# miniufo/xcontour

Measured on AMD Instinct MI355X. Metric: lat-lon cells*contours/s, full Keff pipeline, higher is better.
Workload: dtype f64

## Files before the change

### xcontour_amd/csrc/xc_capi.h

```cpp
#pragma once
#include "xc_internal.h"
#include <assert.h>

namespace xc {

inline size_t al(size_t x) { return (x + 255) & ~(size_t)255; }
inline size_t esize(int dtype) { return dtype == XC_F32 ? 4 : 8; }
inline size_t dA_bytes(int rank, int64_t nslab, int64_t ny, int64_t nx)
{
    return rank == XC_DA_ROW ? (size_t)ny * 8 : rank == XC_DA_PLANE ? (size_t)ny * nx * 8 : rank == XC_DA_SLAB ? (size_t)nslab * ny * nx * 8 : 0;
}

#define XC_TRY(expr) do { int _rc = (expr); if (_rc != XC_OK) return _rc; } while (0)
#define XC_CTX(ctx) do { if (!(ctx)) return xc::fail(nullptr, XC_EBADARG, "null context"); \
                         hipError_t _e = hipSetDevice((ctx)->device); \
                         if (_e != hipSuccess) return xc::hipfail((ctx), _e, "hipSetDevice"); } while (0)

int grow(xc_ctx* ctx, void** p, size_t* have, size_t need);
void mm_touch(xc_ctx* ctx, const void* p, size_t bytes);
const void* resident_lookup(const xc_ctx* ctx, const void* h, size_t n);
int hist_ev_begin(xc_ctx* ctx);
int hist_ev_end(xc_ctx* ctx);

int h2d(xc_ctx* ctx, void* d, const void* h, size_t n);
int stage_in(xc_ctx* ctx, void* slot, const void* h, size_t n, const void** dev);
int stage_small(xc_ctx* ctx, void* slot, const void* h, size_t n, const void** dev);
int flush_in(xc_ctx* ctx);
int d2h(xc_ctx* ctx, void* h, const void* d, size_t n);
void* out_direct(xc_ctx* ctx, void* h, size_t n);

struct Stage {
    struct Out { void* host; const void* dev; size_t bytes; };
// ... 16 lines not shown
```

### xcontour_amd/csrc/xc_comm.hip

```cpp
#include "xc_internal.h"
#include <dlfcn.h>
#include <string.h>

namespace xc {
namespace {

struct UniqueId { char internal[128]; };
typedef void* Comm;
typedef int (*fn_get_id)(UniqueId*);
typedef int (*fn_init_rank)(Comm*, int, UniqueId, int);
typedef int (*fn_allgather)(const void*, void*, size_t, int , Comm, hipStream_t);
typedef int (*fn_destroy)(Comm);
typedef const char* (*fn_errstr)(int);
typedef int (*fn_sendrecv)(void*, size_t, int , int , Comm, hipStream_t);
typedef int (*fn_group)(void);
typedef int (*fn_comm_int)(const Comm, int*);
typedef int (*fn_version)(int*);

struct Rccl {
    void* h = nullptr;
    fn_get_id get_id = nullptr; fn_init_rank init_rank = nullptr; fn_allgather allgather = nullptr;
    fn_destroy destroy = nullptr; fn_errstr errstr = nullptr;
    fn_sendrecv send = nullptr, recv = nullptr; fn_group group_start = nullptr, group_end = nullptr; fn_destroy abort = nullptr;
    fn_comm_int count = nullptr, user_rank = nullptr, cu_device = nullptr; fn_version version = nullptr;
// ... 47 lines not shown
{
    if (ctx->comm_stream) return XC_OK;
    XC_HIP(ctx, hipStreamCreateWithFlags(&ctx->comm_stream, hipStreamNonBlocking));
    XC_HIP(ctx, hipEventCreateWithFlags(&ctx->ev_comm_in, hipEventDisableTiming));
    XC_HIP(ctx, hipEventCreateWithFlags(&ctx->ev_comm_out, hipEventDisableTiming));
    return XC_OK;
}

}
}

using namespace xc;

#define XC_COMM_CTX(ctx) do { if (!(ctx)) return fail(nullptr, XC_EBADARG, "null context"); \
                              hipError_t _e = hipSetDevice((ctx)->device); \
                              if (_e != hipSuccess) return hipfail((ctx), _e, "hipSetDevice"); } while (0)

extern "C" {

int xc_comm_unique_id(xc_ctx* ctx, void* out_id128)
{
    if (!ctx || !out_id128) return fail(ctx, XC_EBADARG, "xc_comm_unique_id: bad arguments");
    int rc = load_rccl(ctx); if (rc != XC_OK) return rc;
    UniqueId id;
    const int r = g_rccl.get_id(&id);
    if (r != 0) return rccl_fail(ctx, r, "ncclGetUniqueId");
    memcpy(out_id128, &id, sizeof(id));
    return XC_OK;
}

int xc_comm_create(int device, int nranks, int rank, const void* id128, void** out_comm, char* err, size_t errlen)
// ... 61 lines not shown
    }
    if (!ctx->comm) return XC_OK;
    int v = 0;
    if (g_rccl.count && g_rccl.count(ctx->comm, &v) == 0) out->comm_count = v;
    if (g_rccl.user_rank && g_rccl.user_rank(ctx->comm, &v) == 0) out->comm_rank = v;
    if (g_rccl.cu_device && g_rccl.cu_device(ctx->comm, &v) == 0) out->comm_device = v;
    return XC_OK;
}

int xc_comm_allgather_dev(xc_ctx* ctx, const void* send, void* recv, size_t bytes_per_rank)
{
    if (!ctx || !ctx->comm) return fail(ctx, XC_EBADARG, "xc_comm_allgather: no communicator (call xc_comm_init)");
    if (!send || !recv) return fail(ctx, XC_EBADARG, "xc_comm_allgather: NULL buffer");
    hipError_t e = hipSetDevice(ctx->device);
    if (e != hipSuccess) return hipfail(ctx, e, "hipSetDevice");
    const int r = g_rccl.allgather(send, recv, bytes_per_rank, 0 , ctx->comm, ctx->stream);
    if (r != 0) return rccl_fail(ctx, r, "ncclAllGather");
    return XC_OK;
}

int xc_comm_gather_dev(xc_ctx* ctx, const void* send, size_t bytes, void* recv, size_t rank_stride, int root)
{
    XC_COMM_CTX(ctx);
    if (!ctx->comm) return fail(ctx, XC_EBADARG, "xc_comm_gather: no communicator (call xc_comm_init)");
    if (!g_rccl.send || !g_rccl.recv || !g_rccl.group_start || !g_rccl.group_end)
        return fail(ctx, XC_EHIP, "xc_comm_gather: librccl lacks ncclSend / ncclRecv / ncclGroupStart / ncclGroupEnd");
    if (!send || root < 0 || root >= ctx->comm_nranks || (ctx->comm_rank == root && !recv) || rank_stride < bytes)
        return fail(ctx, XC_EBADARG, "xc_comm_gather: bad arguments");
    { const int rc = ensure_comm_stream(ctx); if (rc != XC_OK) return rc; }
    if (bytes == 0) return XC_OK;
// ... 97 lines not shown

int xc_comm_abort(xc_ctx* ctx)
{
    if (!ctx) return fail(nullptr, XC_EBADARG, "null context");
    if (ctx->comm) {
        Comm c = ctx->comm; ctx->comm = nullptr;
        if (g_rccl.abort) { const int r = g_rccl.abort(c); if (r != 0) return rccl_fail(ctx, r, "ncclCommAbort"); }
    }
    return XC_OK;
}

int xc_comm_finalize(xc_ctx* ctx)
{
    if (!ctx) return fail(nullptr, XC_EBADARG, "null context");
    if (ctx->comm) {
        (void)hipStreamSynchronize(ctx->stream);
        if (ctx->comm_stream) (void)hipStreamSynchronize(ctx->comm_stream);
        const int r = g_rccl.destroy(ctx->comm);
        ctx->comm = nullptr;
        if (r != 0) return rccl_fail(ctx, r, "ncclCommDestroy");
    }
    return XC_OK;
}

}
```

### xcontour_amd/csrc/xc_context.hip

```cpp
#include "xc_capi.h"
#include <string.h>
#include <stdio.h>
#include <stdlib.h>
#include <new>
#include <mutex>
#include <set>
#include <utility>

namespace xc {

static thread_local std::string g_err;

int fail(xc_ctx* ctx, int code, const std::string& msg)
{
    if (ctx) {
        ctx->err = msg;
        ctx->pending_out.clear(); ctx->pending_in.clear(); ctx->pin_in_off = 0; ctx->pin_out_off = 0;
        for (auto& e : ctx->small_in) if (e.epoch == ctx->small_epoch) { e.host.clear(); e.epoch = ~0ull; }
        ++ctx->small_epoch;
    } else g_err = msg;
    return code;
}

int hipfail(xc_ctx* ctx, hipError_t e, const char* what)
{
    std::string m = std::string("HIP error: ") + hipGetErrorString(e) + " in " + what;
    (void)hipGetLastError();
    return fail(ctx, e == hipErrorOutOfMemory ? XC_ENOMEM : XC_EHIP, m);
}

int grow(xc_ctx* ctx, void** p, size_t* have, size_t need)
{
    if (need <= *have) return XC_OK;
    size_t want = *have ? *have : (size_t)1 << 20;
    while (want < need) want *= 2;
    if (*p) {
        XC_HIP(ctx, hipStreamSynchronize(ctx->stream));
        XC_HIP(ctx, hipFree(*p));
        *p = nullptr; *have = 0;
    }
    hipError_t e = hipMalloc(p, want);
    if (e != hipSuccess) { want = need; e = hipMalloc(p, want); }
    if (e != hipSuccess) return hipfail(ctx, e, "hipMalloc(scratch)");
    *have = want;
    return XC_OK;
}

int ensure_scratch(xc_ctx* ctx, size_t bytes) { return grow(ctx, &ctx->scratch, &ctx->scratch_bytes, bytes); }
int ensure_arena(xc_ctx* ctx, size_t bytes)   { return grow(ctx, &ctx->arena, &ctx->arena_bytes, bytes); }
int ensure_big(xc_ctx* ctx, size_t bytes)     { return grow(ctx, &ctx->big, &ctx->big_bytes, bytes); }

int ensure_ones(xc_ctx* ctx, size_t n)
// ... 94 lines not shown
    }
    if (strncmp(prop.gcnArchName, "gfx950", 6) != 0) {
        std::string m = std::string("xc_create: device is ") + prop.gcnArchName + ", this library is built for gfx950 only";
        delete ctx; return fail(nullptr, XC_ENODEV, m);
    }
    snprintf(ctx->name, sizeof(ctx->name), "%s (%s, %d CUs, %.0f GB)", prop.name[0] ? prop.name : "AMD Instinct [name not reported by the driver]",
             prop.gcnArchName, prop.multiProcessorCount, (double)prop.totalGlobalMem / 1e9);
    {
        auto env_int = [](const char* name, int dflt) { const char* e = getenv(name); return e ? atoi(e) : dflt; };
        HistKnobs& k = ctx->knobs;
        k.xcd_map = env_int("XC_HIST_XCDMAP", 1); k.tile_map = env_int("XC_HIST_TILEMAP", 1); k.vec4 = env_int("XC_HIST_VEC4", -1); k.e32 = env_int("XC_HIST_E32", 1);
        k.threads = env_int("XC_HIST_THREADS", 0); k.ncopy = env_int("XC_HIST_NCOPY", 0); k.rows = env_int("XC_HIST_ROWS", 0);
        k.bps = env_int("XC_HIST_BPS", 0);
        k.cross_ncopy = env_int("XC_CROSS_NCOPY", 0); k.cross_blocks = env_int("XC_CROSS_BLOCKS", 0);
        k.copy_kernel = env_int("XC_COPY_KERNEL", 1); k.copy_out_kb = env_int("XC_COPY_OUT_KB", 256); if (k.copy_out_kb < 1 || k.copy_out_kb > 1024) k.copy_out_kb = 256; k.single = env_int("XC_KEFF_SINGLE", 1); k.single_timeout_us = env_int("XC_KEFF_SINGLE_TIMEOUT_US", 50000); k.single_map = env_int("XC_KEFF_SINGLE_MAP", 0);
        k.sort_range = env_int("XC_SORT_RANGE", 1); k.lwa_fast = env_int("XC_LWA_FAST", 1); k.k1_nt = env_int("XC_K1_NT", 0); k.lwa_strip = env_int("XC_LWA_STRIP", 1);
    }
    ctx->cus = prop.multiProcessorCount;
    if ((e = hipStreamCreateWithFlags(&ctx->stream, hipStreamNonBlocking)) != hipSuccess) {
        int rc = hipfail(nullptr, e, "hipStreamCreate"); delete ctx; return rc;
    }
    if ((e = hipStreamCreateWithFlags(&ctx->copy_stream, hipStreamNonBlocking)) != hipSuccess ||
        (e = hipEventCreateWithFlags(&ctx->ev_copy, hipEventDisableTiming)) != hipSuccess ||
        (e = hipEventCreateWithFlags(&ctx->ev_compute, hipEventDisableTiming)) != hipSuccess) {
        int rc = hipfail(nullptr, e, "hipStreamCreate(copy)"); delete ctx; return rc;
    }
    if ((e = hipEventCreate(&ctx->ev_hist0)) != hipSuccess || (e = hipEventCreate(&ctx->ev_hist1)) != hipSuccess) {
        int rc = hipfail(nullptr, e, "hipEventCreate"); delete ctx; return rc;
    }
    *out = ctx;
    return XC_OK;
}

int xc_destroy(xc_ctx* ctx)
{
    if (!ctx) return XC_OK;
    (void)hipSetDevice(ctx->device);
    (void)xc_comm_finalize(ctx);
    if (ctx->copy_stream) (void)hipStreamSynchronize(ctx->copy_stream);
    if (ctx->stream) (void)hipStreamSynchronize(ctx->stream);
    if (ctx->comm_stream) { (void)hipStreamSynchronize(ctx->comm_stream); (void)hipStreamDestroy(ctx->comm_stream); }
    if (ctx->ev_comm_in) (void)hipEventDestroy(ctx->ev_comm_in);
    if (ctx->ev_comm_out) (void)hipEventDestroy(ctx->ev_comm_out);
    if (ctx->pinned_flag) (void)hipHostFree(ctx->pinned_flag);
    for (auto& e : ctx->small_in) if (e.dev) (void)hipFree(e.dev);
    if (ctx->pin_in) (void)hipHostFree(ctx->pin_in);
    if (ctx->pin_out) (void)hipHostFree(ctx->pin_out);
    if (ctx->lwa_flag) (void)hipFree(ctx->lwa_flag);
    if (ctx->single_ws) (void)hipFree(ctx->single_ws);
    if (ctx->single_stamps) (void)hipFree(ctx->single_stamps);
    for (auto& e : ctx->resident) (void)hipFree(e.dev);
    if (ctx->ev_copy) (void)hipEventDestroy(ctx->ev_copy);
    if (ctx->ev_compute) (void)hipEventDestroy(ctx->ev_compute);
    if (ctx->copy_stream) (void)hipStreamDestroy(ctx->copy_stream);
    if (ctx->scratch) (void)hipFree(ctx->scratch);
// ... 10 lines not shown

int xc_device_name(xc_ctx* ctx, char* buf, size_t buflen)
{
    if (!ctx || !buf || buflen == 0) return fail(ctx, XC_EBADARG, "xc_device_name: bad arguments");
    snprintf(buf, buflen, "%s", ctx->name);
    return XC_OK;
}

int xc_device_cus(xc_ctx* ctx, int* out_cus)
{
    if (!ctx || !out_cus) return fail(ctx, XC_EBADARG, "xc_device_cus: bad arguments");
    *out_cus = ctx->cus;
    return XC_OK;
}

void* xc_stream(xc_ctx* ctx) { return ctx ? (void*)ctx->stream : nullptr; }

int xc_malloc(xc_ctx* ctx, size_t bytes, void** out_dptr)
{
    XC_CTX(ctx);
    if (!out_dptr) return fail(ctx, XC_EBADARG, "xc_malloc: out is NULL");
    *out_dptr = nullptr;
    XC_HIP(ctx, hipMalloc(out_dptr, bytes ? bytes : 1));
    return XC_OK;
}

int xc_keep_resident(xc_ctx* ctx, const void* host_ptr, size_t bytes)
{
    XC_CTX(ctx);
    if (!host_ptr || bytes == 0) return fail(ctx, XC_EBADARG, "xc_keep_resident: bad arguments");
    XC_HIP(ctx, hipStreamSynchronize(ctx->copy_stream));
// ... 192 lines not shown
```

### xcontour_amd/csrc/xc_forms.hip

```cpp
#include "xc_capi.h"
#include <cmath>

using namespace xc;

static bool check_ascending(const double* contours, int64_t nc, int ncont)
{
    for (int64_t s = 0; s < nc; ++s)
        for (int k = 0; k < ncont; ++k) {
            const double c = contours[s * ncont + k];
            if (c != c || (k > 0 && c < contours[s * ncont + k - 1])) return false;
        }
    return true;
}

static int clen_recorded(xc_ctx* ctx, int rc)
{
    if (rc != XC_OK) ctx->last_clen = xc_clen_geometry{};
    return rc;
}

static int contour_lengths_host(xc_ctx* ctx, const void* q, int q_dtype, int64_t nslab, int64_t ny, int64_t nx,
                                const double* ycoord, const double* xcoord, double radius,
                                const double* contours, int ncont, int contours_per_slab,
                                double* out_len, uint64_t* out_nseg)
// ... 299 lines not shown

int xc_set_lwa_exact(xc_ctx* ctx, int exact)
{
    if (!ctx) return fail(nullptr, XC_EBADARG, "null context");
    if (exact < 0 || exact > 3) return fail(ctx, XC_EBADARG, "xc_set_lwa_exact: mode must be 0 (automatic), 1 (band walk), 2 (interval kernel, checked) or 3 (interval kernel, premises vouched for)");
    ctx->lwa_exact = exact;
    return XC_OK;
}

int xc_last_lwa_path(xc_ctx* ctx, int* out_path)
{
    if (!ctx || !out_path) return fail(ctx, XC_EBADARG, "xc_last_lwa_path: bad arguments");
    if (ctx->last_lwa_path < 0) {
        unsigned f = 0;
        XC_HIP(ctx, hipSetDevice(ctx->device));
        XC_HIP(ctx, hipMemcpyAsync(&f, ctx->lwa_flag, sizeof(f), hipMemcpyDeviceToHost, ctx->stream));
        XC_HIP(ctx, hipStreamSynchronize(ctx->stream));
        ctx->last_lwa_path = (f == ctx->lwa_epoch) ? 2 : 1;
    }
    *out_path = ctx->last_lwa_path;
    return XC_OK;
}

int xc_last_sort_path(xc_ctx* ctx, int* out_path)
{
    if (!ctx || !out_path) return fail(ctx, XC_EBADARG, "xc_last_sort_path: bad arguments");
    *out_path = ctx->last_sort_path;
    return XC_OK;
}

// ... 10 lines not shown
```

### xcontour_amd/csrc/xc_hist_det.hip

```cpp
#include "xc_internal.h"

namespace xc {

namespace {

#include "xc_hist_kernel.h"

template <typename TQ, int VEC, int NINT, bool GRAD>
int det3_two(xc_ctx* ctx, const HistGeom& g, int64_t nslab, const HistArgs& a)
{
    const bool da2d = a.dA_rank == XC_DA_PLANE || a.dA_rank == XC_DA_SLAB;
    if constexpr (GRAD && NINT == 0 && VEC == 2) {
        if (da2d && a.periodic_x && a.dA_pos_finite && !a.negate && !a.last_closed)
            return a.q_next ? launch_three<TQ, VEC, NINT, GRAD, true, true, true, 3>(ctx, g, nslab, a)
                            : launch_three<TQ, VEC, NINT, GRAD, true, false, true, 3>(ctx, g, nslab, a);
    }
    if constexpr ((GRAD && NINT == 0) || (!GRAD && NINT == 1)) {
        if (a.q_next)
            return da2d ? launch_three<TQ, VEC, NINT, GRAD, true, true, false, 3>(ctx, g, nslab, a)
                        : launch_three<TQ, VEC, NINT, GRAD, false, true, false, 3>(ctx, g, nslab, a);
    }
    if (a.q_next) return fail(ctx, XC_EBADARG, "xc_hist: q_next rides in the Keff layouts only");
    return da2d ? launch_three<TQ, VEC, NINT, GRAD, true, false, false, 3>(ctx, g, nslab, a)
                : launch_three<TQ, VEC, NINT, GRAD, false, false, false, 3>(ctx, g, nslab, a);
// ... 55 lines not shown

}

int det_limbs_total(int nch) { return det_total_limbs(nch); }

int launch_hist_det3(xc_ctx* ctx, int q_dtype, int nint, int grad, const HistGeom& g, int64_t nslab, const HistArgs& a)
{
    if (g.vec == 4) return fail(ctx, XC_EBADARG, "xc_hist: no four-cell variant with deterministic sums");
    if (!a.part_c || !a.det_c0_out) return fail(ctx, XC_EBADARG, "xc_hist: the one-pass deterministic sums need the count partials and the window constants");
    if (q_dtype == XC_F64) return g.vec == 2 ? det3_one<double, 2>(ctx, nint, grad, g, nslab, a) : det3_one<double, 1>(ctx, nint, grad, g, nslab, a);
    if (q_dtype == XC_F32) return g.vec == 2 ? det3_one<float, 2>(ctx, nint, grad, g, nslab, a) : det3_one<float, 1>(ctx, nint, grad, g, nslab, a);
    return fail(ctx, XC_EBADARG, "xc_hist: q_dtype must be XC_F32 or XC_F64");
}

int launch_det3_reduce(xc_ctx* ctx, int64_t nslab, int bps, int nch, int nbin, const double* part_l, const unsigned* part_c,
                       const int* c0, double* red_h, unsigned long long* red_c)
{
    dim3 grid((unsigned)((nch * nbin + 7) / 8), (unsigned)nslab);
    hipLaunchKernelGGL(k_det3_reduce, grid, dim3(256), 0, ctx->stream, reinterpret_cast<const unsigned long long*>(part_l), part_c,
                       bps, nch, nbin, c0, red_h, red_c);
    XC_HIP(ctx, hipGetLastError());
    return XC_OK;
}

}
```

### xcontour_amd/csrc/xc_internal.h

```cpp
#pragma once
#include <hip/hip_runtime.h>
#include <stdint.h>
#include <stddef.h>
#include <string>
#include <type_traits>
#include <vector>
#include "../../include/xcontour_hip.h"

struct HistKnobs {
    int copy_out_kb = 256;
    int copy_kernel = 1;
    int xcd_map = 1;
    int tile_map = 1;
    int vec4 = -1;
    int e32 = 1;
    int threads = 0;
    int ncopy = 0;
    int rows = 0;
    int bps = 0;
    int cross_ncopy = 0, cross_blocks = 0;
    int k1_nt = 0;
    int lwa_fast = 1;
    int lwa_strip = 1;
    int sort_range = 1;
    int single = 1;
    int single_timeout_us = 50000;
    int single_map = 0;
};

struct xc_ctx {
    int device = 0;
    HistKnobs knobs;
    hipStream_t stream = nullptr;
    hipStream_t copy_stream = nullptr;
    hipStream_t comm_stream = nullptr;
    hipEvent_t ev_comm_in = nullptr, ev_comm_out = nullptr;
    hipEvent_t ev_copy = nullptr, ev_compute = nullptr;
    unsigned* pinned_flag = nullptr;
    char* pin_in = nullptr;  size_t pin_in_off = 0;
    char* pin_out = nullptr; size_t pin_out_off = 0;
    struct PendingOut { void* host; const void* pinned; size_t bytes; const void* dev; };
    std::vector<PendingOut> pending_out;
// ... 8 lines not shown
    int cus = 0;
    char name[256] = {0};
    std::string err;
    void*  scratch = nullptr;   size_t scratch_bytes = 0;
    void*  arena = nullptr;     size_t arena_bytes = 0;
    double* ones = nullptr;     size_t ones_n = 0;
    void*  big = nullptr;       size_t big_bytes = 0;
    int timing = 0;
    hipEvent_t ev_hist0 = nullptr, ev_hist1 = nullptr;
    int ev_valid = 0;
    void* comm = nullptr; int comm_nranks = 0, comm_rank = 0;
    hipEvent_t user_ev0 = nullptr, user_ev1 = nullptr;
    double* mmnext[2] = {nullptr, nullptr};  size_t mmnext_bytes[2] = {0, 0};
    int mm_cur = 0, mm_valid = 0, mm_P = 0, mm_dtype = 0;
    const void* mm_q = nullptr;  int64_t mm_nslab = 0, mm_ny = 0, mm_nx = 0;  int mm_gen = 0;
    int lwa_exact = 0;
    int last_lwa_path = 0;
    unsigned lwa_epoch = 0;
    unsigned* lwa_flag = nullptr;
    int last_sort_path = 0;
    void* single_ws = nullptr;  unsigned single_launches = 0;  int single_dirty_bins[2] = {0, 0};
    int last_keff_path = 0;
    xc_hist_variant last_hist = {};
    xc_clen_geometry last_clen = {};
    unsigned long long* single_stamps = nullptr;
};

namespace xc {

int fail(xc_ctx* ctx, int code, const std::string& msg);
int ensure_big_lds(xc_ctx* ctx, const void* kernel, int bytes);
int hipfail(xc_ctx* ctx, hipError_t e, const char* what);

#define XC_HIP(ctx, call)                                                     \
    do {                                                                      \
        hipError_t _e = (call);                                               \
        if (_e != hipSuccess) return xc::hipfail((ctx), _e, #call);           \
    } while (0)

int ensure_scratch(xc_ctx* ctx, size_t bytes);
int ensure_arena(xc_ctx* ctx, size_t bytes);
int ensure_ones(xc_ctx* ctx, size_t n);
int ensure_big(xc_ctx* ctx, size_t bytes);

constexpr int kMinmaxBlocks = 2048;
// ... 130 lines not shown
                     int dA_rank, SingleGeom* g);
int launch_keff_single(xc_ctx* ctx, int q_dtype, const SingleArgs& a, const SingleGeom& g);

int launch_minmax_partial(xc_ctx* ctx, const void* q, int q_dtype, int64_t nslab, int64_t ncell, double* part,
                          double* zero = nullptr, int64_t nzero = 0, bool finite_only = false);
struct SmallCopies { const void* src[8]; void* dst[8]; unsigned bytes[8]; };
int launch_copy_small(xc_ctx* ctx, const SmallCopies& c, int count);
int launch_minmax_final(xc_ctx* ctx, const double* part, int64_t nslab, int P, double* out);
int launch_levels(xc_ctx* ctx, const double* minmax, int q_dtype, int64_t nslab, int N, int increase,
                  int ctr_dtype, int right_edge, double* ctr, double* edges, int32_t* status, int P = 0, double* minmax_out = nullptr);
int hist_geometry(xc_ctx* ctx, int q_dtype, int64_t nslab, int64_t ny, int64_t nx, int nbin, int nch,
                  const void* q, HistGeom* g, int keff_fast_layout = 0, int det = 0);
int launch_hist(xc_ctx* ctx, int q_dtype, int nint, int grad, const HistGeom& g, int64_t nslab, const HistArgs& a);
int launch_hist_det3(xc_ctx* ctx, int q_dtype, int nint, int grad, const HistGeom& g, int64_t nslab, const HistArgs& a);
int launch_det3_reduce(xc_ctx* ctx, int64_t nslab, int bps, int nch, int nbin, const double* part_l, const unsigned* part_c,
                       const int* c0, double* red_h, unsigned long long* red_c);
int det_limbs_total(int nch);
int launch_finalize(xc_ctx* ctx, int64_t nslab, const FinalArgs& a);
int launch_rowsum(xc_ctx* ctx, const void* mask, int mask_dtype, const double* dA, int dA_rank,
                  int64_t ny, int64_t nx, int multiply, double* out_rows);
int launch_grad2(xc_ctx* ctx, const void* q, int q_dtype, int64_t nslab, int64_t ny, int64_t nx,
                 const double* rdx, const double* rdy, int periodic_x, double* out);
int launch_lwa(xc_ctx* ctx, const void* q, int q_dtype, const double* Q, const double* coord,
               const double* dA, int dA_rank, double dA_max, const double* M, int M_rank,
               int64_t nslab, int64_t ny, int64_t nx, int increase, int part, int variant,
               const int32_t* mask_idx, int nmask, double* out_lwa, int8_t* out_masks);
size_t sort_workspace_bytes(int64_t n, int64_t nslab);
struct SortArgs {
    const void*   q;     int q_dtype;
    const void*   mask;  int mask_dtype, mask_per_slab;
    const double* dA;    int dA_rank;
    int64_t       nslab, ny, nx;
    int           negate;
// ... 23 lines not shown
```

### xcontour_amd/csrc/xc_keff.hip

```cpp
#include "xc_capi.h"
#include <string.h>

using namespace xc;

static const void* vec_align_bits(const void* q, int q_dtype, const void* q_next, const double* dA, int dA_rank,
                                  const void* const* integ, const int32_t* integ_dtype, int nint)
{
    uintptr_t bits = reinterpret_cast<uintptr_t>(q) | reinterpret_cast<uintptr_t>(q_next);
    auto need16 = [&](const void* p) {
        const uintptr_t a = reinterpret_cast<uintptr_t>(p);
        if (a % 16 != 0) bits |= (q_dtype == XC_F32) ? 4 : 8;
    };
    if (dA && (dA_rank == XC_DA_PLANE || dA_rank == XC_DA_SLAB)) need16(dA);
    for (int i = 0; i < nint; ++i) {
        if (integ_dtype[i] == XC_F64) need16(integ[i]);
        else if (reinterpret_cast<uintptr_t>(integ[i]) % 8 != 0) bits |= (q_dtype == XC_F32) ? 4 : 8;
    }
    return reinterpret_cast<const void*>(bits);
}

static int check_hist_desc(xc_ctx* ctx, const xc_hist_desc* d)
{
    if (!d) return fail(ctx, XC_EBADARG, "xc_hist: desc is NULL");
    if (!d->q || !d->edges) return fail(ctx, XC_EBADARG, "xc_hist: q / edges is NULL");
// ... 17 lines not shown
    size_t o_ph, o_pc, o_rh, o_rc, o_c0, o_dp, o_dm, pair_bytes, total = 0;  char* base = nullptr;
    size_t put(size_t bytes) { const size_t at = total; total += al(bytes); return at; }
    K3Scratch(int64_t nslab, int bps, int nch, int nbin, int det, bool minmax_partials, bool part_h = true)
    {
        const size_t S = (size_t)nslab, mmb = S * kMinmaxBlocks * 2 * sizeof(double);
        put(minmax_partials ? mmb : 0);
        o_ph = put(part_h ? S * bps * (det ? det_limbs_total(nch) : nch) * nbin * sizeof(double) : 0);
        o_pc = put(S * bps * nbin * sizeof(unsigned));
        o_rh = put(S * nch * nbin * sizeof(double));
        o_rc = put(S * nbin * sizeof(unsigned long long));
        o_c0 = put(det ? S * nch * sizeof(int) : 0);
        o_dp = put(det ? mmb : 0);
        pair_bytes = al(S * 2 * sizeof(double));
        o_dm = put(det ? (3 + XC_MAX_INTEGRANDS) * pair_bytes : 0);
    }
    int reserve(xc_ctx* ctx) { XC_TRY(ensure_scratch(ctx, total)); base = (char*)ctx->scratch; return XC_OK; }
    double*   mmpart() const { return (double*)base; }
    double*   part_h() const { return (double*)(base + o_ph); }
    unsigned* part_c() const { return (unsigned*)(base + o_pc); }
    size_t    part_c_bytes() const { return o_rh - o_pc; }
    double*   red_h() const  { return (double*)(base + o_rh); }
    unsigned long long* red_c() const { return (unsigned long long*)(base + o_rc); }
    int64_t   acc_words() const { return (int64_t)((o_c0 - o_rh) / 8); }
    int*      c0() const     { return (int*)(base + o_c0); }
    double*   det_part() const { return (double*)(base + o_dp); }
    double*   det_pair(int i) const { return (double*)(base + o_dm + i * pair_bytes); }
};

template <typename Desc, typename Args>
static int set_weights(xc_ctx* ctx, const Desc* d, Args& a)
{
// ... 18 lines not shown
    return XC_OK;
}

static void keff_final(FinalArgs& f, const xc_keff_desc* d, int vstride, int ntbl)
{
    f.lt = d->lt; f.reverse = !d->increase;
    f.keff = 1; f.ctr_f32 = d->ctr_dtype == XC_F32; f.ctr = d->ctr; f.vstride = vstride;
    f.tbl = d->tbl; f.tbl_coord = d->tbl_coord; f.ntbl = ntbl;
    f.preY = d->preY; f.npre = d->interp ? d->npre : 0;
    f.nkeff_mask = d->nkeff_mask; f.lmin_scale = d->lmin_scale;
    f.o_area = d->area; f.o_intS = d->intgrdS; f.o_latEq = d->latEq; f.o_dqdA = d->dqdA; f.o_dSdA = d->dintSdA;
    f.o_Leq2 = d->Leq2; f.o_Lmin = d->Lmin; f.o_nkeff = d->nkeff; f.o_interp = d->interp;
}

static int det_one_pass(xc_ctx* ctx, int q_dtype, int nint, int grad, const HistGeom& g, int64_t nslab, int64_t ny, int64_t nx,
                        HistArgs& a, const K3Scratch& L, double dA_max_host, const void* const* integ, const int* integ_dtype, FinalArgs& f)
{
    double* part = L.det_part();
    auto extrema = [&](const void* p, int dtype, int64_t ns, int64_t ncell, double* out) -> int {
        XC_TRY(launch_minmax_partial(ctx, p, dtype, ns, ncell, part, nullptr, 0, true));
        return launch_minmax_final(ctx, part, ns, minmax_blocks(ncell, ns), out);
    };
    a.det_dA_max = -1.0; a.det_dA_max_dev = nullptr; a.det_dA_stride = 0;
    if (dA_max_host > 0.0 && dA_max_host < __builtin_inf()) a.det_dA_max = dA_max_host;
    else if (a.dA == ctx->ones) a.det_dA_max = 1.0;
    else {
        double* out = L.det_pair(0);
        const int64_t ns = a.dA_rank == XC_DA_SLAB ? nslab : 1, ncell = a.dA_rank == XC_DA_ROW ? ny : ny * nx;
        XC_TRY(extrema(a.dA, XC_F64, ns, ncell, out));
        a.det_dA_max_dev = out; a.det_dA_stride = a.dA_rank == XC_DA_SLAB ? 1 : 0;
    }
    a.det_q_mm = nullptr;
    if (grad && !a.levels_mode) {
        double* out = L.det_pair(1);
        XC_TRY(extrema(a.q, q_dtype, nslab, ny * nx, out));
        a.det_q_mm = out;
    }
    for (int i = 0; i < nint; ++i) {
        double* out = L.det_pair(2 + i);
        XC_TRY(extrema(integ[i], integ_dtype[i], nslab, ny * nx, out));
        a.det_int_mm[i] = out;
    }
    a.det_c0_out = L.c0();
    XC_TRY(launch_hist_det3(ctx, q_dtype, nint, grad, g, nslab, a));
    XC_TRY(launch_det3_reduce(ctx, nslab, g.bps, f.nch, f.nbin, a.part_h, a.part_c, L.c0(), f.red_h, f.red_c));
    f.skip_reduce = 1;
    return XC_OK;
}

static int hist_recorded(xc_ctx* ctx, int rc)
{
    if (rc != XC_OK && ctx) ctx->last_hist = xc_hist_variant{};
    return rc;
}

static int hist_dev(xc_ctx* ctx, const xc_hist_desc* d)
{
    XC_TRY(check_hist_desc(ctx, d));
    const int nbin = (int)(d->nedge - 1), nch = 1 + d->nint + (d->grad ? 1 : 0);
    HistGeom g;
// ... 91 lines not shown
    keff_final(f, d, vstride, (int)d->ny);
    f.abort_flag = &a.cur->abort; f.status_out = d->status;
    f.dbg = ctx->single_stamps ? ctx->single_stamps + 8 : nullptr;
    ctx->mm_valid = 0;
    XC_TRY(hist_ev_begin(ctx));
    XC_TRY(launch_keff_single(ctx, d->q_dtype, a, g));
    XC_TRY(hist_ev_end(ctx));
    XC_TRY(launch_finalize(ctx, d->nslab, f));
    ctx->single_dirty_bins[cur] = N;
    ctx->single_dirty_bins[1u - cur] = 0;
    ++ctx->single_launches;
    ctx->last_keff_path = 1;
    return XC_OK;
}

static int keff_dev(xc_ctx* ctx, const xc_keff_desc* d)
{
    if (!d) return fail(ctx, XC_EBADARG, "xc_keff: desc is NULL");
    if (!d->q || !d->ctr || !d->area || !d->tbl || !d->tbl_coord) return fail(ctx, XC_EBADARG, "xc_keff: q/ctr/area/tbl/tbl_coord must be given");
    if (d->q_dtype != XC_F32 && d->q_dtype != XC_F64) return fail(ctx, XC_EBADARG, "xc_keff: bad q_dtype");
    if (d->ctr_dtype != XC_F32 && d->ctr_dtype != XC_F64) return fail(ctx, XC_EBADARG, "xc_keff: bad ctr_dtype");
    if (d->nslab < 1 || d->ny < 2 || d->nx < 1 || d->N < 2) return fail(ctx, XC_EBADARG, "xc_keff: need nslab>=1, ny>=2, nx>=1, N>=2");
    if (d->dA_rank < XC_DA_NONE || d->dA_rank > XC_DA_SLAB || (d->dA_rank != XC_DA_NONE && !d->dA)) return fail(ctx, XC_EBADARG, "xc_keff: bad dA");
    if (d->grad ? (!d->rdx || !d->rdy) : !d->grdS) return fail(ctx, XC_EBADARG, "xc_keff: need rdx/rdy (grad=1) or grdS (grad=0)");
    if (d->npre < 0 || (d->npre > 0 && d->interp && !d->preY)) return fail(ctx, XC_EBADARG, "xc_keff: preY is NULL");
    if (d->out_stride != 0 && d->out_stride < d->N) return fail(ctx, XC_EBADARG, "xc_keff: out_stride must be 0 (dense) or >= N");
    const int vstride = d->out_stride ? d->out_stride : d->N;
    const int N = d->N, nch = 2;
    const int det = d->deterministic ? 1 : 0;
    const void* q_next = d->q_next;
    ctx->last_keff_path = 0;
    if (d->single_read != XC_SINGLE_NEVER && ctx->knobs.single != 0 && !det && d->grad &&
        d->nslab <= (d->single_read == XC_SINGLE_FORCE ? kSingleMaxSlabs : 1)) {
        const int rc = keff_single(ctx, d);
        if (rc != XC_EAGAIN) return rc;
    }
    HistGeom g;
    {
        const void* gi[1] = {d->grdS}; const int32_t gt[1] = {d->grdS_dtype};
        const bool da2d = d->dA_rank == XC_DA_PLANE || d->dA_rank == XC_DA_SLAB;
        const bool fast_layout = d->grad && da2d && d->periodic_x && d->dA_pos_finite && d->right_edge != XC_EDGE_NUMPY;
        const bool supplied_f32 = !d->grad && da2d && d->q_dtype == XC_F32 && d->grdS_dtype == XC_F32 &&
                                  reinterpret_cast<uintptr_t>(d->grdS) % 16 == 0;
        XC_TRY(hist_geometry(ctx, d->q_dtype, d->nslab, d->ny, d->nx, N, nch,
                             vec_align_bits(d->q, d->q_dtype, d->q_next, d->dA, d->dA_rank, gi, gt, d->grad ? 0 : 1), &g,
                             fast_layout ? 1 : (supplied_f32 ? 2 : 0), det));
    }
    K3Scratch L(d->nslab, g.bps, nch, N, det, true);
    XC_TRY(L.reserve(ctx));
    double* mmpart = L.mmpart();
    int mmP = minmax_blocks(d->ny * d->nx, d->nslab);
    bool accum = false;

    if (ctx->mm_valid && ctx->mm_q == d->q && ctx->mm_nslab == d->nslab && ctx->mm_ny == d->ny &&
        ctx->mm_nx == d->nx && ctx->mm_dtype == d->q_dtype && ctx->mm_gen == d->q_gen) {
        mmpart = ctx->mmnext[ctx->mm_cur]; mmP = ctx->mm_P;
    } else {
        accum = !det && g.bps > 64;
        XC_TRY(launch_minmax_partial(ctx, d->q, d->q_dtype, d->nslab, d->ny * d->nx, mmpart,
                                     accum ? L.red_h() : nullptr, accum ? L.acc_words() : 0));
    }
    ctx->mm_valid = 0;
    double* mm_next = nullptr;
    if (q_next) {
// ... 4 lines not shown

    HistArgs a; memset(&a, 0, sizeof(a));
    FinalArgs f; memset(&f, 0, sizeof(f));
    XC_TRY(hist_common(ctx, d, nch, N, g, L, a, f));
    if (!d->grad) { a.integ[0] = d->grdS; a.integ_f32[0] = d->grdS_dtype == XC_F32; }
    a.q_next = q_next; a.mm_next = mm_next;
    a.mmpart = mmpart; a.P = mmP; a.levels_mode = 1;
    a.last_closed = d->right_edge == XC_EDGE_NUMPY;
    a.increase = d->increase; a.ctr_f32 = d->ctr_dtype == XC_F32;
    a.right_edge = d->right_edge; a.inv_nm1 = 1.0 / (double)(N - 1);
    a.ctr_out = d->ctr; a.ctr_stride = vstride; a.status = d->status;
    if (accum) { a.acc_h = f.red_h; a.acc_c = d->counts ? f.red_c : nullptr; f.skip_reduce = 1; }
    XC_TRY(hist_ev_begin(ctx));
    if (det) {
        const void* gi[1] = {d->grdS}; const int gt[1] = {d->grdS_dtype};
        XC_TRY(det_one_pass(ctx, d->q_dtype, d->grad ? 0 : 1, d->grad, g, d->nslab, d->ny, d->nx, a, L, d->dA_max, gi, gt, f));
    } else {
        XC_TRY(launch_hist(ctx, d->q_dtype, d->grad ? 0 : 1, d->grad, g, d->nslab, a));
    }
    XC_TRY(hist_ev_end(ctx));
    if (q_next) {
        ctx->mm_cur = 1 - ctx->mm_cur; ctx->mm_valid = 1; ctx->mm_P = g.bps; ctx->mm_q = q_next;
        ctx->mm_nslab = d->nslab; ctx->mm_ny = d->ny; ctx->mm_nx = d->nx; ctx->mm_dtype = d->q_dtype;
        ctx->mm_gen = d->q_gen;
    }

    keff_final(f, d, vstride, (int)d->ny);
    return launch_finalize(ctx, d->nslab, f);
}

extern "C" {

int xc_minmax_dev(xc_ctx* ctx, const void* q, int q_dtype, int64_t nslab, int64_t ncell, double* out_minmax)
{
    XC_CTX(ctx);
    if (!q || !out_minmax || nslab < 1 || ncell < 1) return fail(ctx, XC_EBADARG, "xc_minmax: bad arguments");
    XC_TRY(ensure_scratch(ctx, al((size_t)nslab * kMinmaxBlocks * 2 * sizeof(double))));
    double* part = (double*)ctx->scratch;
    XC_TRY(launch_minmax_partial(ctx, q, q_dtype, nslab, ncell, part));
    return launch_minmax_final(ctx, part, nslab, minmax_blocks(ncell, nslab), out_minmax);
}

int xc_minmax(xc_ctx* ctx, const void* q, int q_dtype, int64_t nslab, int64_t ncell, double* out_minmax)
// ... 120 lines not shown
    double* host[8] = {area, intgrdS, latEq, dqdA, dintSdA, Leq2, Lmin, nkeff};
    double* o[8]; for (int i = 0; i < 8; ++i) o[i] = st.keep(host[i], vb);
    double* di = npre > 0 ? st.out(interp, ib) : nullptr;
    XC_TRY(h2d(ctx, dp, pdf, pb)); XC_TRY(h2d(ctx, dc, ctr, vb));
    XC_TRY(h2d(ctx, dt, tbl, tb)); XC_TRY(h2d(ctx, dy, tbl_coord, tb));
    if (dpre) { if (!preY) return fail(ctx, XC_EBADARG, "xc_keff_epilogue: preY is NULL"); XC_TRY(h2d(ctx, dpre, preY, yb)); }
    XC_TRY(flush_in(ctx));
    XC_TRY(xc_keff_epilogue_dev(ctx, dp, dc, ctr_dtype, nslab, N, increase, lt, dt, dy, ntbl, dpre, npre, nkeff_mask, lmin_scale,
                                o[0], o[1], o[2], o[3], o[4], o[5], o[6], o[7], di));
    XC_TRY(st.deliver());
    return xc_sync(ctx);
}

int xc_keff_dev(xc_ctx* ctx, const xc_keff_desc* d)
{
    XC_CTX(ctx);
    ctx->last_hist = xc_hist_variant{};
    return hist_recorded(ctx, keff_dev(ctx, d));
}

int xc_last_keff_path(xc_ctx* ctx, int* out_path)
{
    if (!ctx || !out_path) return fail(ctx, XC_EBADARG, "xc_last_keff_path: bad arguments");
    *out_path = ctx->last_keff_path;
    return XC_OK;
}

int xc_dbg_single_stamps(xc_ctx* ctx, int enable, void** out_dev, int* out_slots)
{
    XC_CTX(ctx);
    if (ctx->single_stamps) { XC_HIP(ctx, hipStreamSynchronize(ctx->stream)); (void)hipFree(ctx->single_stamps); ctx->single_stamps = nullptr; }
// ... 19 lines not shown
```

### xcontour_amd/csrc/xc_misc.hip

```cpp
#include "xc_internal.h"

namespace xc {

namespace {

__device__ __forceinline__ double dnan() { return __longlong_as_double(0x7ff8000000000000LL); }
__device__ __forceinline__ double dinf() { return __longlong_as_double(0x7ff0000000000000LL); }

template <typename T> struct V16;
template <> struct V16<double> { using type = double2; static constexpr int n = 2; typedef double ext __attribute__((ext_vector_type(2))); };
template <> struct V16<float>  { using type = float4;  static constexpr int n = 4; typedef float ext __attribute__((ext_vector_type(4))); };
template <typename T>
__device__ __forceinline__ typename V16<T>::type ld16_nt(const typename V16<T>::type* p)
{
    const typename V16<T>::ext t = __builtin_nontemporal_load(reinterpret_cast<const typename V16<T>::ext*>(p));
    typename V16<T>::type r;
    if constexpr (V16<T>::n == 2) { r.x = t.x; r.y = t.y; } else { r.x = t.x; r.y = t.y; r.z = t.z; r.w = t.w; }
    return r;
}

__device__ __forceinline__ void mm(double& mn, double& mx, double v) { mn = fmin(mn, v); mx = fmax(mx, v); }
__device__ __forceinline__ void mmv(double& mn, double& mx, const double2& v) { mm(mn, mx, v.x); mm(mn, mx, v.y); }
__device__ __forceinline__ void mmv(double& mn, double& mx, const float4& v)
{
// ... 285 lines not shown
    return XC_OK;
}

int launch_levels(xc_ctx* ctx, const double* minmax, int q_dtype, int64_t nslab, int N, int increase,
                  int ctr_dtype, int right_edge, double* ctr, double* edges, int32_t* status, int P, double* minmax_out)
{
    if (!minmax || !ctr || !edges || !status || N < 2 || nslab < 1)
        return fail(ctx, XC_EBADARG, "xc_levels: bad arguments (need N >= 2)");
    const double inv = 1.0 / (double)(N - 1);
    hipLaunchKernelGGL(k_levels, dim3((unsigned)nslab), dim3(256), 0, ctx->stream, minmax, P, minmax_out, N, increase,
                       q_dtype == XC_F32, ctr_dtype == XC_F32, right_edge, inv, ctr, edges, status);
    XC_HIP(ctx, hipGetLastError());
    return XC_OK;
}

int launch_finalize(xc_ctx* ctx, int64_t nslab, const FinalArgs& a_in)
{
    FinalArgs a = a_in;
    if (a.vstride <= 0) a.vstride = a.nbin;
    hipStream_t st = ctx->stream;
    size_t lds = ((size_t)2 * a.nch * a.nbin + (a.keff ? 7 * (size_t)a.nbin : 0)) * sizeof(double);
    a.big = nullptr; a.big_stride = 0;
    if (lds > kLdsBudget) {
        a.big_stride = lds / sizeof(double);
        const int rc = ensure_big(ctx, (size_t)nslab * lds);
        if (rc != XC_OK) return rc;
        a.big = (double*)ctx->big;
        lds = 0;
    }
    { const int rc = ensure_big_lds(ctx, reinterpret_cast<const void*>(k_finalize), (int)kLdsBudget + 4096); if (rc != XC_OK) return rc; }
    a.tbl_in_lds = 0;
    if (!a.big && a.keff && lds + (size_t)2 * a.ntbl * sizeof(double) <= 64 * 1024) {
        a.tbl_in_lds = 1;
        lds += (size_t)2 * a.ntbl * sizeof(double);
    }
// ... 97 lines not shown
```

Baseline: 72290 billion.

## Run Keff finalize epilogue on a high-priority side stream overlapping next chunk

When a Keff call has a following chunk (q_next), the det reduce and finalize kernels are launched on a separate high-priority stream, ordered by events, so they can overlap the next call's histogram work. The scratch area is double-buffered across two sets, and output address ranges are tracked so that a later call which does not continue the chain, or which touches those outputs, joins the epilogue first. Every other API entry point joins the side stream before doing its work. This adds event and stream overhead and bookkeeping, and risks hazards if the aliasing checks are incomplete.

```diff
diff --git a/xcontour_amd/csrc/xc_capi.h b/xcontour_amd/csrc/xc_capi.h
--- a/xcontour_amd/csrc/xc_capi.h
+++ b/xcontour_amd/csrc/xc_capi.h
@@ -12,10 +12,12 @@
 }
 
 #define XC_TRY(expr) do { int _rc = (expr); if (_rc != XC_OK) return _rc; } while (0)
-#define XC_CTX(ctx) do { if (!(ctx)) return xc::fail(nullptr, XC_EBADARG, "null context"); \
-                         hipError_t _e = hipSetDevice((ctx)->device); \
-                         if (_e != hipSuccess) return xc::hipfail((ctx), _e, "hipSetDevice"); } while (0)
+#define XC_CTX_NOJOIN(ctx) do { if (!(ctx)) return xc::fail(nullptr, XC_EBADARG, "null context"); \
+                                hipError_t _e = hipSetDevice((ctx)->device); \
+                                if (_e != hipSuccess) return xc::hipfail((ctx), _e, "hipSetDevice"); } while (0)
+#define XC_CTX(ctx) do { XC_CTX_NOJOIN(ctx); XC_TRY(xc::join_epilogue(ctx)); } while (0)
 
+int ensure_epilogue_stream(xc_ctx* ctx);
 int grow(xc_ctx* ctx, void** p, size_t* have, size_t need);
 void mm_touch(xc_ctx* ctx, const void* p, size_t bytes);
 const void* resident_lookup(const xc_ctx* ctx, const void* h, size_t n);
diff --git a/xcontour_amd/csrc/xc_comm.hip b/xcontour_amd/csrc/xc_comm.hip
--- a/xcontour_amd/csrc/xc_comm.hip
+++ b/xcontour_amd/csrc/xc_comm.hip
@@ -85,7 +85,8 @@
 
 #define XC_COMM_CTX(ctx) do { if (!(ctx)) return fail(nullptr, XC_EBADARG, "null context"); \
                               hipError_t _e = hipSetDevice((ctx)->device); \
-                              if (_e != hipSuccess) return hipfail((ctx), _e, "hipSetDevice"); } while (0)
+                              if (_e != hipSuccess) return hipfail((ctx), _e, "hipSetDevice"); \
+                              const int _rc = join_epilogue(ctx); if (_rc != XC_OK) return _rc; } while (0)
 
 extern "C" {
 
@@ -177,6 +178,7 @@
     if (!send || !recv) return fail(ctx, XC_EBADARG, "xc_comm_allgather: NULL buffer");
     hipError_t e = hipSetDevice(ctx->device);
     if (e != hipSuccess) return hipfail(ctx, e, "hipSetDevice");
+    { const int rc = join_epilogue(ctx); if (rc != XC_OK) return rc; }
     const int r = g_rccl.allgather(send, recv, bytes_per_rank, 0 , ctx->comm, ctx->stream);
     if (r != 0) return rccl_fail(ctx, r, "ncclAllGather");
     return XC_OK;
@@ -304,6 +306,7 @@
 {
     if (!ctx) return fail(nullptr, XC_EBADARG, "null context");
     if (ctx->comm) {
+        (void)join_epilogue(ctx);
         (void)hipStreamSynchronize(ctx->stream);
         if (ctx->comm_stream) (void)hipStreamSynchronize(ctx->comm_stream);
         const int r = g_rccl.destroy(ctx->comm);
diff --git a/xcontour_amd/csrc/xc_context.hip b/xcontour_amd/csrc/xc_context.hip
--- a/xcontour_amd/csrc/xc_context.hip
+++ b/xcontour_amd/csrc/xc_context.hip
@@ -15,6 +15,9 @@
 {
     if (ctx) {
         ctx->err = msg;
+        for (int s = 0; s < 2; ++s)
+            if (ctx->epi_busy[s]) { ctx->epi_busy[s] = 0; if (hipStreamWaitEvent(ctx->stream, ctx->ev_epi_done[s], 0) != hipSuccess) (void)hipGetLastError(); }
+        ctx->epi_lo = ctx->epi_hi = nullptr;
         ctx->pending_out.clear(); ctx->pending_in.clear(); ctx->pin_in_off = 0; ctx->pin_out_off = 0;
         for (auto& e : ctx->small_in) if (e.epoch == ctx->small_epoch) { e.host.clear(); e.epoch = ~0ull; }
         ++ctx->small_epoch;
@@ -29,6 +32,30 @@
     return fail(ctx, e == hipErrorOutOfMemory ? XC_ENOMEM : XC_EHIP, m);
 }
 
+int join_epilogue(xc_ctx* ctx)
+{
+    for (int s = 0; s < 2; ++s)
+        if (ctx->epi_busy[s]) {
+            ctx->epi_busy[s] = 0;
+            XC_HIP(ctx, hipStreamWaitEvent(ctx->stream, ctx->ev_epi_done[s], 0));
+        }
+    ctx->epi_lo = ctx->epi_hi = nullptr;
+    return XC_OK;
+}
+
+int ensure_epilogue_stream(xc_ctx* ctx)
+{
+    if (ctx->epi_stream) return XC_OK;
+    int lo = 0, hi = 0;
+    XC_HIP(ctx, hipDeviceGetStreamPriorityRange(&lo, &hi));
+    XC_HIP(ctx, hipStreamCreateWithPriority(&ctx->epi_stream, hipStreamNonBlocking, hi));
+    for (int s = 0; s < 2; ++s) {
+        XC_HIP(ctx, hipEventCreateWithFlags(&ctx->ev_hist_done[s], hipEventDisableTiming));
+        XC_HIP(ctx, hipEventCreateWithFlags(&ctx->ev_epi_done[s], hipEventDisableTiming));
+    }
+    return XC_OK;
+}
+
 int grow(xc_ctx* ctx, void** p, size_t* have, size_t need)
 {
     if (need <= *have) return XC_OK;
@@ -36,6 +63,7 @@
     while (want < need) want *= 2;
     if (*p) {
         XC_HIP(ctx, hipStreamSynchronize(ctx->stream));
+        if (ctx->epi_stream) XC_HIP(ctx, hipStreamSynchronize(ctx->epi_stream));
         XC_HIP(ctx, hipFree(*p));
         *p = nullptr; *have = 0;
     }
@@ -160,6 +188,7 @@
         k.bps = env_int("XC_HIST_BPS", 0);
         k.cross_ncopy = env_int("XC_CROSS_NCOPY", 0); k.cross_blocks = env_int("XC_CROSS_BLOCKS", 0);
         k.copy_kernel = env_int("XC_COPY_KERNEL", 1); k.copy_out_kb = env_int("XC_COPY_OUT_KB", 256); if (k.copy_out_kb < 1 || k.copy_out_kb > 1024) k.copy_out_kb = 256; k.single = env_int("XC_KEFF_SINGLE", 1); k.single_timeout_us = env_int("XC_KEFF_SINGLE_TIMEOUT_US", 50000); k.single_map = env_int("XC_KEFF_SINGLE_MAP", 0);
+        k.epi_stream = env_int("XC_KEFF_EPILOGUE_STREAM", 1);
         k.sort_range = env_int("XC_SORT_RANGE", 1); k.lwa_fast = env_int("XC_LWA_FAST", 1); k.k1_nt = env_int("XC_K1_NT", 0); k.lwa_strip = env_int("XC_LWA_STRIP", 1);
     }
     ctx->cus = prop.multiProcessorCount;
@@ -185,6 +214,11 @@
     (void)xc_comm_finalize(ctx);
     if (ctx->copy_stream) (void)hipStreamSynchronize(ctx->copy_stream);
     if (ctx->stream) (void)hipStreamSynchronize(ctx->stream);
+    if (ctx->epi_stream) { (void)hipStreamSynchronize(ctx->epi_stream); (void)hipStreamDestroy(ctx->epi_stream); }
+    for (int s = 0; s < 2; ++s) {
+        if (ctx->ev_hist_done[s]) (void)hipEventDestroy(ctx->ev_hist_done[s]);
+        if (ctx->ev_epi_done[s]) (void)hipEventDestroy(ctx->ev_epi_done[s]);
+    }
     if (ctx->comm_stream) { (void)hipStreamSynchronize(ctx->comm_stream); (void)hipStreamDestroy(ctx->comm_stream); }
     if (ctx->ev_comm_in) (void)hipEventDestroy(ctx->ev_comm_in);
     if (ctx->ev_comm_out) (void)hipEventDestroy(ctx->ev_comm_out);
@@ -225,7 +259,12 @@
     return XC_OK;
 }
 
-void* xc_stream(xc_ctx* ctx) { return ctx ? (void*)ctx->stream : nullptr; }
+void* xc_stream(xc_ctx* ctx)
+{
+    if (!ctx) return nullptr;
+    (void)join_epilogue(ctx);
+    return (void*)ctx->stream;
+}
 
 int xc_malloc(xc_ctx* ctx, size_t bytes, void** out_dptr)
 {
diff --git a/xcontour_amd/csrc/xc_forms.hip b/xcontour_amd/csrc/xc_forms.hip
--- a/xcontour_amd/csrc/xc_forms.hip
+++ b/xcontour_amd/csrc/xc_forms.hip
@@ -337,6 +337,7 @@
     if (ctx->last_lwa_path < 0) {
         unsigned f = 0;
         XC_HIP(ctx, hipSetDevice(ctx->device));
+        XC_TRY(join_epilogue(ctx));
         XC_HIP(ctx, hipMemcpyAsync(&f, ctx->lwa_flag, sizeof(f), hipMemcpyDeviceToHost, ctx->stream));
         XC_HIP(ctx, hipStreamSynchronize(ctx->stream));
         ctx->last_lwa_path = (f == ctx->lwa_epoch) ? 2 : 1;
diff --git a/xcontour_amd/csrc/xc_hist_det.hip b/xcontour_amd/csrc/xc_hist_det.hip
--- a/xcontour_amd/csrc/xc_hist_det.hip
+++ b/xcontour_amd/csrc/xc_hist_det.hip
@@ -93,10 +93,10 @@
 }
 
 int launch_det3_reduce(xc_ctx* ctx, int64_t nslab, int bps, int nch, int nbin, const double* part_l, const unsigned* part_c,
-                       const int* c0, double* red_h, unsigned long long* red_c)
+                       const int* c0, double* red_h, unsigned long long* red_c, hipStream_t st)
 {
     dim3 grid((unsigned)((nch * nbin + 7) / 8), (unsigned)nslab);
-    hipLaunchKernelGGL(k_det3_reduce, grid, dim3(256), 0, ctx->stream, reinterpret_cast<const unsigned long long*>(part_l), part_c,
+    hipLaunchKernelGGL(k_det3_reduce, grid, dim3(256), 0, st ? st : ctx->stream, reinterpret_cast<const unsigned long long*>(part_l), part_c,
                        bps, nch, nbin, c0, red_h, red_c);
     XC_HIP(ctx, hipGetLastError());
     return XC_OK;
diff --git a/xcontour_amd/csrc/xc_internal.h b/xcontour_amd/csrc/xc_internal.h
--- a/xcontour_amd/csrc/xc_internal.h
+++ b/xcontour_amd/csrc/xc_internal.h
@@ -26,6 +26,7 @@
     int single = 1;
     int single_timeout_us = 50000;
     int single_map = 0;
+    int epi_stream = 1;
 };
 
 struct xc_ctx {
@@ -64,6 +65,12 @@
     double* mmnext[2] = {nullptr, nullptr};  size_t mmnext_bytes[2] = {0, 0};
     int mm_cur = 0, mm_valid = 0, mm_P = 0, mm_dtype = 0;
     const void* mm_q = nullptr;  int64_t mm_nslab = 0, mm_ny = 0, mm_nx = 0;  int mm_gen = 0;
+    hipStream_t epi_stream = nullptr;
+    hipEvent_t ev_hist_done[2] = {nullptr, nullptr}, ev_epi_done[2] = {nullptr, nullptr};
+    int epi_set = 0;
+    int epi_busy[2] = {0, 0};
+    size_t epi_total = 0;
+    const char* epi_lo = nullptr;  const char* epi_hi = nullptr;
     int lwa_exact = 0;
     int last_lwa_path = 0;
     unsigned lwa_epoch = 0;
@@ -79,6 +86,7 @@
 namespace xc {
 
 int fail(xc_ctx* ctx, int code, const std::string& msg);
+int join_epilogue(xc_ctx* ctx);
 int ensure_big_lds(xc_ctx* ctx, const void* kernel, int bytes);
 int hipfail(xc_ctx* ctx, hipError_t e, const char* what);
 
@@ -239,9 +247,9 @@
 int launch_hist(xc_ctx* ctx, int q_dtype, int nint, int grad, const HistGeom& g, int64_t nslab, const HistArgs& a);
 int launch_hist_det3(xc_ctx* ctx, int q_dtype, int nint, int grad, const HistGeom& g, int64_t nslab, const HistArgs& a);
 int launch_det3_reduce(xc_ctx* ctx, int64_t nslab, int bps, int nch, int nbin, const double* part_l, const unsigned* part_c,
-                       const int* c0, double* red_h, unsigned long long* red_c);
+                       const int* c0, double* red_h, unsigned long long* red_c, hipStream_t st = nullptr);
 int det_limbs_total(int nch);
-int launch_finalize(xc_ctx* ctx, int64_t nslab, const FinalArgs& a);
+int launch_finalize(xc_ctx* ctx, int64_t nslab, const FinalArgs& a, hipStream_t st = nullptr);
 int launch_rowsum(xc_ctx* ctx, const void* mask, int mask_dtype, const double* dA, int dA_rank,
                   int64_t ny, int64_t nx, int multiply, double* out_rows);
 int launch_grad2(xc_ctx* ctx, const void* q, int q_dtype, int64_t nslab, int64_t ny, int64_t nx,
diff --git a/xcontour_amd/csrc/xc_keff.hip b/xcontour_amd/csrc/xc_keff.hip
--- a/xcontour_amd/csrc/xc_keff.hip
+++ b/xcontour_amd/csrc/xc_keff.hip
@@ -55,7 +55,7 @@
         pair_bytes = al(S * 2 * sizeof(double));
         o_dm = put(det ? (3 + XC_MAX_INTEGRANDS) * pair_bytes : 0);
     }
-    int reserve(xc_ctx* ctx) { XC_TRY(ensure_scratch(ctx, total)); base = (char*)ctx->scratch; return XC_OK; }
+    int reserve(xc_ctx* ctx, int sets = 1, int set = 0) { XC_TRY(ensure_scratch(ctx, sets * total)); base = (char*)ctx->scratch + set * total; return XC_OK; }
     double*   mmpart() const { return (double*)base; }
     double*   part_h() const { return (double*)(base + o_ph); }
     unsigned* part_c() const { return (unsigned*)(base + o_pc); }
@@ -104,7 +104,8 @@
 }
 
 static int det_one_pass(xc_ctx* ctx, int q_dtype, int nint, int grad, const HistGeom& g, int64_t nslab, int64_t ny, int64_t nx,
-                        HistArgs& a, const K3Scratch& L, double dA_max_host, const void* const* integ, const int* integ_dtype, FinalArgs& f)
+                        HistArgs& a, const K3Scratch& L, double dA_max_host, const void* const* integ, const int* integ_dtype, FinalArgs& f,
+                        bool reduce_now = true)
 {
     double* part = L.det_part();
     auto extrema = [&](const void* p, int dtype, int64_t ns, int64_t ncell, double* out) -> int {
@@ -133,7 +134,7 @@
     }
     a.det_c0_out = L.c0();
     XC_TRY(launch_hist_det3(ctx, q_dtype, nint, grad, g, nslab, a));
-    XC_TRY(launch_det3_reduce(ctx, nslab, g.bps, f.nch, f.nbin, a.part_h, a.part_c, L.c0(), f.red_h, f.red_c));
+    if (reduce_now) XC_TRY(launch_det3_reduce(ctx, nslab, g.bps, f.nch, f.nbin, a.part_h, a.part_c, L.c0(), f.red_h, f.red_c));
     f.skip_reduce = 1;
     return XC_OK;
 }
@@ -255,6 +256,37 @@
     return XC_OK;
 }
 
+static void epilogue_range(const xc_keff_desc* d, const char** lo, const char** hi)
+{
+    const size_t S = (size_t)d->nslab, vstride = d->out_stride ? d->out_stride : d->N;
+    const size_t vb = ((S - 1) * vstride + d->N) * sizeof(double);
+    *lo = *hi = nullptr;
+    auto add = [&](const void* p, size_t bytes) {
+        if (!p || !bytes) return;
+        const char* c = (const char*)p;
+        if (!*lo || c < *lo) *lo = c;
+        if (!*hi || c + bytes > *hi) *hi = c + bytes;
+    };
+    const double* v[9] = {d->ctr, d->area, d->intgrdS, d->latEq, d->dqdA, d->dintSdA, d->Leq2, d->Lmin, d->nkeff};
+    for (const double* p : v) add(p, vb);
+    add(d->counts, S * d->N * sizeof(uint64_t));
+    if (d->npre > 0) add(d->interp, S * 9 * d->npre * sizeof(double));
+}
+
+static bool continues_chain(const xc_ctx* ctx, const xc_keff_desc* d)
+{
+    if (!d || !d->q_next || !ctx->knobs.epi_stream || !(ctx->epi_busy[0] || ctx->epi_busy[1])) return false;
+    if (!(ctx->mm_valid && ctx->mm_q == d->q && ctx->mm_nslab == d->nslab && ctx->mm_ny == d->ny && ctx->mm_nx == d->nx &&
+          ctx->mm_dtype == d->q_dtype && ctx->mm_gen == d->q_gen)) return false;
+    if (!d->ctr || d->nslab < 1 || d->N < 2 || (d->out_stride != 0 && d->out_stride < d->N)) return false;
+    const size_t S = (size_t)d->nslab, vstride = d->out_stride ? d->out_stride : d->N;
+    auto clear_of = [&](const void* p, size_t bytes) {
+        const char* c = (const char*)p;
+        return !p || !ctx->epi_lo || c + bytes <= ctx->epi_lo || c >= ctx->epi_hi;
+    };
+    return clear_of(d->ctr, ((S - 1) * vstride + d->N) * sizeof(double)) && clear_of(d->status, S * sizeof(int32_t));
+}
+
 static int keff_dev(xc_ctx* ctx, const xc_keff_desc* d)
 {
     if (!d) return fail(ctx, XC_EBADARG, "xc_keff: desc is NULL");
@@ -273,6 +305,7 @@
     ctx->last_keff_path = 0;
     if (d->single_read != XC_SINGLE_NEVER && ctx->knobs.single != 0 && !det && d->grad &&
         d->nslab <= (d->single_read == XC_SINGLE_FORCE ? kSingleMaxSlabs : 1)) {
+        XC_TRY(join_epilogue(ctx));
         const int rc = keff_single(ctx, d);
         if (rc != XC_EAGAIN) return rc;
     }
@@ -288,7 +321,15 @@
                              fast_layout ? 1 : (supplied_f32 ? 2 : 0), det));
     }
     K3Scratch L(d->nslab, g.bps, nch, N, det, true);
-    XC_TRY(L.reserve(ctx));
+    const bool overlap = q_next && ctx->knobs.epi_stream != 0;
+    if (!overlap || L.total != ctx->epi_total) XC_TRY(join_epilogue(ctx));
+    const int set = overlap ? ctx->epi_set : 0;
+    if (overlap) {
+        XC_TRY(ensure_epilogue_stream(ctx));
+        XC_TRY(L.reserve(ctx, 2, set));
+        ctx->epi_total = L.total;
+        if (ctx->epi_busy[set]) XC_HIP(ctx, hipStreamWaitEvent(ctx->stream, ctx->ev_epi_done[set], 0));
+    } else XC_TRY(L.reserve(ctx));
     double* mmpart = L.mmpart();
     int mmP = minmax_blocks(d->ny * d->nx, d->nslab);
     bool accum = false;
@@ -323,7 +364,7 @@
     XC_TRY(hist_ev_begin(ctx));
     if (det) {
         const void* gi[1] = {d->grdS}; const int gt[1] = {d->grdS_dtype};
-        XC_TRY(det_one_pass(ctx, d->q_dtype, d->grad ? 0 : 1, d->grad, g, d->nslab, d->ny, d->nx, a, L, d->dA_max, gi, gt, f));
+        XC_TRY(det_one_pass(ctx, d->q_dtype, d->grad ? 0 : 1, d->grad, g, d->nslab, d->ny, d->nx, a, L, d->dA_max, gi, gt, f, !overlap));
     } else {
         XC_TRY(launch_hist(ctx, d->q_dtype, d->grad ? 0 : 1, d->grad, g, d->nslab, a));
     }
@@ -335,7 +376,18 @@
     }
 
     keff_final(f, d, vstride, (int)d->ny);
-    return launch_finalize(ctx, d->nslab, f);
+    if (!overlap) return launch_finalize(ctx, d->nslab, f);
+    XC_HIP(ctx, hipEventRecord(ctx->ev_hist_done[set], ctx->stream));
+    XC_HIP(ctx, hipStreamWaitEvent(ctx->epi_stream, ctx->ev_hist_done[set], 0));
+    int rc = det ? launch_det3_reduce(ctx, d->nslab, g.bps, f.nch, f.nbin, a.part_h, a.part_c, L.c0(), f.red_h, f.red_c, ctx->epi_stream) : XC_OK;
+    if (rc == XC_OK) rc = launch_finalize(ctx, d->nslab, f, ctx->epi_stream);
+    XC_HIP(ctx, hipEventRecord(ctx->ev_epi_done[set], ctx->epi_stream));
+    ctx->epi_busy[set] = 1; ctx->epi_set = 1 - set;
+    const char *lo, *hi;
+    epilogue_range(d, &lo, &hi);
+    if (!ctx->epi_lo || lo < ctx->epi_lo) ctx->epi_lo = lo;
+    if (!ctx->epi_hi || hi > ctx->epi_hi) ctx->epi_hi = hi;
+    return rc;
 }
 
 extern "C" {
@@ -486,7 +538,8 @@
 
 int xc_keff_dev(xc_ctx* ctx, const xc_keff_desc* d)
 {
-    XC_CTX(ctx);
+    XC_CTX_NOJOIN(ctx);
+    if (!continues_chain(ctx, d)) XC_TRY(join_epilogue(ctx));
     ctx->last_hist = xc_hist_variant{};
     return hist_recorded(ctx, keff_dev(ctx, d));
 }
diff --git a/xcontour_amd/csrc/xc_misc.hip b/xcontour_amd/csrc/xc_misc.hip
--- a/xcontour_amd/csrc/xc_misc.hip
+++ b/xcontour_amd/csrc/xc_misc.hip
@@ -323,11 +323,11 @@
     return XC_OK;
 }
 
-int launch_finalize(xc_ctx* ctx, int64_t nslab, const FinalArgs& a_in)
+int launch_finalize(xc_ctx* ctx, int64_t nslab, const FinalArgs& a_in, hipStream_t st)
 {
     FinalArgs a = a_in;
     if (a.vstride <= 0) a.vstride = a.nbin;
-    hipStream_t st = ctx->stream;
+    if (!st) st = ctx->stream;
     size_t lds = ((size_t)2 * a.nch * a.nbin + (a.keff ? 7 * (size_t)a.nbin : 0)) * sizeof(double);
     a.big = nullptr; a.big_stride = 0;
     if (lds > kLdsBudget) {
```

After: 71740 billion. Within noise of the previous version (-0.8%).
